# OSU-NLP-Group/saev

Hardware: AMD Instinct MI355X
Metric: activations/sec (train step), d_in=1024 x32 k=32 (higher is better)
Workload: dtype f32 (encoder: fp16 MFMA first pass with a rigorous error margin, survivors recomputed exactly in fp32; all else fp32)

## Files before the change

### include/saev_amd.h

```cpp
#ifndef SAEV_AMD_H
#define SAEV_AMD_H

#include <stdint.h>

#ifdef __cplusplus
extern "C" {
#endif

#define SAEV_AMD_ABI_VERSION 12

typedef enum {
    SAEV_OK = 0,
    SAEV_INVALID_ARG = -1,
    SAEV_HIP_ERROR = -2,
    SAEV_UNSUPPORTED = -3,
    SAEV_NOT_BOUND = -4,
    SAEV_RCCL_ERROR = -5,
    SAEV_STALE_PARAMS = -6,
    SAEV_ROW_OVERFLOW = -7
} saev_status;

typedef struct {
    int32_t d_model;
    int32_t d_sae;
// ... 44 lines not shown
typedef struct saev_ctx saev_ctx;

typedef struct {
    int32_t struct_size;
    int32_t dw_route;
    int32_t aux_small_max;
    int32_t fwd_route;
    int32_t csc_route;
    int32_t fin_route;
    int32_t prep_route;
    int32_t aux_dense_route;
    int32_t aux_small_route;
    int32_t group_route;
    int32_t aux_split_route;
    int32_t aux_wide_route;
} saev_debug_cfg;

int saev_abi_version(void);
const char* saev_last_error(const saev_ctx* ctx);

int saev_create(const saev_cfg* cfg, int device, saev_ctx** out);
int saev_create_ex(const saev_cfg* cfg, const saev_debug_cfg* dbg, int device, saev_ctx** out);
void saev_destroy(saev_ctx* ctx);

typedef struct {
    int32_t struct_size;
    int32_t row_cap;
    double batch_momentum;
    int32_t list_cap;
    int32_t reserved;
// ... 140 lines not shown
```

### saev_amd/_lib.py

```python

from __future__ import annotations

import ctypes as C
import os
import pathlib

_HERE = pathlib.Path(__file__).resolve().parent
LIB_PATH = pathlib.Path(os.environ.get("SAEV_AMD_LIB", _HERE / "libsaev_amd.so"))

ABI_VERSION = 12


class SaevCfg(C.Structure):
    _fields_ = [
        ("d_model", C.c_int32), ("d_sae", C.c_int32), ("top_k", C.c_int32), ("k_aux", C.c_int32),
        ("alpha", C.c_float), ("dead_threshold_tokens", C.c_int64),
        ("normalize_w_dec", C.c_int32), ("remove_parallel_grads", C.c_int32),
        ("max_batch", C.c_int32), ("encoder_mode", C.c_int32), ("aux_dead_cap", C.c_int32),
        ("shard_world", C.c_int32), ("bound_mode", C.c_int32), ("max_backward_rows", C.c_int32),
        ("activation", C.c_int32),
    ]


class SaevDebugCfg(C.Structure):

    _fields_ = [(n, C.c_int32) for n in ("struct_size", "dw_route", "aux_small_max", "fwd_route", "csc_route", "fin_route", "prep_route", "aux_dense_route",
                                         "aux_small_route", "group_route", "aux_split_route", "aux_wide_route")]


class SaevLayout(C.Structure):
    _fields_ = [(n, C.c_int64) for n in ("off_W_dec", "off_b_dec", "off_W_enc", "off_b_enc", "n_total", "chunk_a", "chunk_b")]


class SaevStepStats(C.Structure):
    _fields_ = [
        ("mse", C.c_float), ("aux", C.c_float), ("l0", C.c_float), ("l1", C.c_float),
        ("grad_norm", C.c_float), ("upper", C.c_float), ("n_dead", C.c_int32),
        ("n_overflow_rows", C.c_int32), ("cand_max", C.c_int32), ("dense_route", C.c_int32), ("sse", C.c_double), ("sum_sq", C.c_double),
    ]


class SaevMuonCfg(C.Structure):
# ... 148 lines not shown
```

### saev_amd/csrc/ctx.hip

```cpp
#include <hip/hip_runtime.h>

#include <algorithm>
#include <cmath>
#include <cstdio>
#include <cstdlib>
#include <cstring>
#include <dlfcn.h>
#include <mutex>
#include <string>
#include <vector>

#include "kernels.h"

namespace {
constexpr int AUX_KSPLIT_MAX = 16;
constexpr int CAND_CAP = 4096;
constexpr int CAND_STRIDE = CAND_CAP + 256;
constexpr int TIMING_RING = 512;
constexpr int DEAD_LAG = 4;
constexpr int DEAD_RING = 16;
enum { AUX_NONE = 0, AUX_SMALL_DEVICE = 1, AUX_SMALL_HOST = 2, AUX_DENSE = 3 };
}

struct saev_ctx {
// ... 42 lines not shown
    float* dval_pairs = nullptr;
    double *sumsq_partials = nullptr, *sumsq_total = nullptr;
    bool wenc_sq_valid = false;
    float2* row_proj = nullptr;
    float* enc_sq = nullptr;
    bool row_proj_valid = false, tail_proj_in_adam = false;
    bool wenc_t_pending = false;
    int64_t* toks = nullptr;
    int32_t *fired = nullptr, *dead = nullptr;
    int32_t* flags = nullptr;
    int32_t *chunk_starts = nullptr, *part_starts = nullptr, *work_latent = nullptr;
    float *dW_encT = nullptr, *partials = nullptr, *db_partials = nullptr;
    bool dws_ok = false;
    int dws_rows = 0;
    bool dws_pairs = false;
    float *gS = nullptr, *xS = nullptr, *dvp = nullptr;
    float* xS_ov = nullptr;
    float* xS_bwd = nullptr;
    float* dval_rows = nullptr;
    bool dval_fwd = false;
    float* wn2 = nullptr;
    float* sq_wave = nullptr;
    int sq_wave_n = 0;
    bool wn2_fresh = false;
    bool dval_pairs_ready = false;
    bool fused_forward = false;
    bool fwd_slices = false;
    bool fwd_step = false;
    float* rs_part = nullptr;
    float* xS_c = nullptr;
// ... 284 lines not shown
    A(dW_encT, S * D); A(partials, (size_t)c->max_part * 2 * D); A(db_partials, c->max_part); A(row_proj, S); A(enc_sq, S);
    {
        const bool rows_only = c->dbg.dw_route == 1;
        c->dws_ok = !rows_only && !btk && D % DWS_SLICE == 0 && (uint64_t)S * D * 4ull < (1ull << 32) && MBB < (1l << 24) &&
                    (uint64_t)MBB * K < (1ull << 31);
    }
    c->fwd_slices = !btk && c->cfg.encoder_mode == SAEV_ENCODER_F16R && c->dbg.fwd_route == 0 && D % RS_SLICE == 0 &&
                    (uint64_t)S * 128ull < (1ull << 32) - 256ull && fused_supported(c->cfg);
    if (c->fwd_slices) {
        A(rs_part, (size_t)(D / RS_SLICE) * MB * REFINE_CAP); A(surv_rng, MB * RS_MAX_RANGES);
        c->rs_lat_range = (int)std::max<long>(RS_LAT_RANGE, ((S + RS_MAX_RANGES - 1) / RS_MAX_RANGES + 255) / 256 * 256);
        c->rs_n_ranges = (int)((S + c->rs_lat_range - 1) / c->rs_lat_range);
    }
    if (c->fwd_slices && !c->dws_ok) A(xS, MBB * D);
    if (c->dws_ok) {
        A(gS, MBB * D); A(xS, MBB * D); A(dvp, (size_t)(D / DWS_SLICE) * MBB * K);
        if (c->dbg.dw_route != 2 && decode_forms_dval((int)D, (int)K)) A(dval_rows, MB * K);
        A(pv, MBB * K); A(pv2, MBB * K); A(plat, MBB * K); A(cut_lat, (MBB * K + DWS_RUN - 1) / DWS_RUN); A(cut_list, 4 * (1 + (MBB * K + DWS_RUN - 1) / DWS_RUN)); A(lat_unused, S);
        if (c->dval_rows != nullptr && c->dbg.fin_route == 0) { A(wn2, S); A(sq_wave, (size_t)2 * dw_slices_waves((int)D, (int)(MBB * K))); }
    }
    A(colsum_partials, ((MBB + 63) / 64) * D);
    A(sumsq_partials, 2 * 1024 + (S + 3) / 4 + 8 + transpose_blocks((int)S, (int)D)); A(sumsq_total, 1);
    if (c->cfg.encoder_mode != SAEV_ENCODER_F32 || KA > 0) {
        c->Dp = (int)((D + 31) / 32 * 32);
        c->S_pad = (int)((S + 255) / 256 * 256);
        c->MB_pad = (int)((MB + 255) / 256 * 256);
        A(zero_bias, std::max(S, D)); A(aux_scales, 16); A(aux_sync, absmax_parts_max((int)MB));
    }
    if (c->cfg.encoder_mode != SAEV_ENCODER_F32) {
        A(xs, (size_t)c->MB_pad * 2 * c->Dp);
// ... 509 lines not shown
                if (c->fwd_step) {
                    RefineSlicesArgs rs{};
                    rs.surv_idx = c->surv_idx; rs.surv_cnt = c->surv_cnt; rs.surv_val = c->surv_val; rs.surv_rng = c->surv_rng;
                    rs.xS = c->xS_c; rs.WeS = c->stream_ok ? c->WeS : c->dW_encT; rs.b_enc = sc.b_enc; rs.part = c->rs_part;
                    rs.n_rows = n; rs.S = c->cfg.d_sae; rs.D = c->cfg.d_model;
                    rs.lat_range = c->rs_lat_range; rs.n_ranges = c->rs_n_ranges;
                    rs.enable_flag = flag; rs.enable_when = when;
                    HIPCHK(c, launch_refine_slices(rs, s));
                    sc.sum_part = c->rs_part; sc.sum_bias = sc.b_enc; sc.sum_n = c->cfg.d_model / RS_SLICE; sc.sum_plane = (size_t)n * REFINE_CAP;
                } else {
                    HIPCHK(c, launch_refine_exact(sc, s));
                }
                sc.row_margin = nullptr; sc.tau_max = nullptr;
                sc.cand_cnt = c->surv_cnt; sc.cand_val = c->surv_val; sc.cand_idx = c->surv_idx; sc.cand_cap = REFINE_CAP; sc.cand_stride = REFINE_CAP;
            }
            HIPCHK(c, launch_select_cand(sc, s));
            return SAEV_OK;
        };
        const bool predict = c->cfg.bound_mode != 0 && ng == 32 && c->cfg.encoder_mode != SAEV_ENCODER_F32;
        int32_t *bad1 = c->flags + 9, *run2 = c->flags + 10, *gate = c->flags + 11;
        if (predict) {
            HIPCHK(c, launch_heur_gate(c->heur_state, pre_flag, gate, s));
            HIPCHK(c, launch_encoder_init(c->cand_cnt, n, c->gmax, 0, s, c->tau_max));
            timing_begin(c, s);
            int rc = run_encoder(c, x, n, EPI_TOPK, nullptr, gate, 0, s, true);
            if (rc != SAEV_OK) return rc;
            timing_end(c, s);
            HIPCHK(c, launch_overflow_check(c->cand_cnt, n, CAND_CAP, gate, bad1, c->flags + 2, c->flags + 3, s, need_dense,
                                            nullptr, c->heur_state + 3, nullptr, pre_flag));
            rc = select_stage(bad1, 0, bad1, c->tau_max);
            if (rc != SAEV_OK) return rc;
// ... 829 lines not shown
        w.part_dec = c->partials; w.part_enc = c->partials + 2 * runs_cap * D;
        w.cut_lat = c->cut_lat; w.cut_list = c->cut_list;
        w.lat_unused = (all_rows && c->fused_step) ? c->lat_unused : nullptr;
        c->unused_valid = w.lat_unused != nullptr;
        w.row_proj = a.row_proj; w.project = a.project; w.enc_sq = a.enc_sq;
        w.clear_bitmap = a.clear_bitmap; w.clear_words = a.clear_words;
        w.have_dval = c->dval_pairs_ready ? 1 : 0;
        c->sq_wave_n = 0;
        if (c->dval_pairs_ready && c->wn2_fresh && part == 0) {
            w.wn2 = c->wn2;
            if (c->fused_step && all_rows && c->sq_wave != nullptr && c->dbg.fin_route != 2) {
                c->sq_wave_n = dw_slices_waves(D, (int)((long)n * K));
                w.sq_wave_dec = c->sq_wave; w.sq_wave_enc = c->sq_wave + c->sq_wave_n;
            }
        }
        HIPCHK(c, launch_dw_slices(w, (int)((long)n * K), part, s));
    } else {
        c->unused_valid = false;
        HIPCHK(c, launch_dw_rows(a, max_work, s));
    }
    if (c->aux_route == AUX_DENSE)
        HIPCHK(c, launch_scatter_add_dead(c->dead_list, c->n_dead_host, D, c->dWd, c->dWe, c->dbe, c->grads + c->off_W_dec,
                                          c->dW_encT, c->grads + c->off_b_enc, lat_lo, lat_hi, s,
                                          c->aux_dev_count ? c->flags + 4 : nullptr, part, a.row_proj, a.W_dec, a.project, a.enc_sq,
                                          c->unused_valid ? c->lat_unused : nullptr, c->sq_wave_n > 0 ? c->starts : nullptr));
    else if (c->aux_route != AUX_NONE)
        HIPCHK(c, launch_scatter_add_dead(c->dead_list, c->aux_mfma ? c->aux_ndp : AUX_SMALL_MAX, D, c->dWd, c->dWe, c->dbe, c->grads + c->off_W_dec,
                                          c->dW_encT, c->grads + c->off_b_enc, lat_lo, lat_hi, s, c->flags + 4, part,
                                          a.row_proj, a.W_dec, a.project, a.enc_sq, c->unused_valid ? c->lat_unused : nullptr,
                                          c->sq_wave_n > 0 ? c->starts : nullptr));
    if (ov && c->aux_route != AUX_NONE && part != 2 && lat_lo == 0)
// ... 549 lines not shown
```

### saev_amd/csrc/kernels.h

```cpp
#pragma once
#include <hip/hip_runtime.h>
#include <stdint.h>

#include <string>

#include "../../include/saev_amd.h"

enum { EPI_DENSE = 0, EPI_TOPK = 1 };

struct EncodeArgs {
    const float* x;
    const float* W_enc;
    const float* b_enc;
    int n_rows, D, S;
    int s_splits;
    float* h_out;
    int ngroups;
    int32_t* gmax;
    int gmax_stride;
    int32_t* cand_cnt;
    float* cand_val;
    int32_t* cand_idx;
    int cand_cap;
    int cand_stride;
// ... 50 lines not shown
    size_t sum_plane;
};
hipError_t launch_refine_exact(const SelectCandArgs& a, hipStream_t stream);
constexpr int REFINE_CAP = 512;
constexpr int RS_SLICE = 32;
constexpr int RS_ROWS_MAX = 8;
constexpr int RS_LAT_RANGE = 32768;
constexpr int RS_MAX_RANGES = 8;
struct RefineSlicesArgs {
    const int32_t* surv_idx; const int32_t* surv_cnt; float* surv_val; const int32_t* surv_rng;
    const float* xS; const float* WeS; const float* b_enc; float* part;
    int n_rows, S, D, lat_range, n_ranges;
    const int32_t* enable_flag; int enable_when;
};
hipError_t launch_refine_slices(const RefineSlicesArgs& a, hipStream_t stream);
hipError_t launch_select_cand(const SelectCandArgs& a, hipStream_t stream);
hipError_t launch_init_i32(int32_t* p, int32_t v, int n, hipStream_t stream);
hipError_t launch_encoder_init(int32_t* cand_cnt, int n_rows, int32_t* gmax, int n_gmax, hipStream_t stream,
                               int32_t* tau_max = nullptr, const int32_t* enable_flag = nullptr, int enable_when = 0);
hipError_t launch_pre_encode(int32_t* cand_cnt, int n_rows, int32_t* gmax, int n_gmax, const float* xnorm, int D,
                             const float* wg_part, int n_part, const float* scales, int32_t* pre_flag, float* wmax_prev,
                             float* margin, int32_t* flags1, hipStream_t stream);
hipError_t launch_heur_gate(float* state, const int32_t* pre_flag, int32_t* gate, hipStream_t stream);
hipError_t launch_heur_update(float* state, const int32_t* bad, const float* cand_mean, int k, const int32_t* gate,
                              hipStream_t stream);
hipError_t launch_step_zero(saev_step_stats* stats, float* upper, int32_t* flag0, hipStream_t stream);
hipError_t launch_wnorm_max(const float* W_encT, int S, int D, float* wg_scratch, float* wmax, hipStream_t stream);
hipError_t launch_f16r_scales(const float* xmax_part, int n_part, const float* wmax, float* scales, hipStream_t stream);
hipError_t launch_pow2_scale(const float* absmax, float* pair, hipStream_t stream);
hipError_t launch_center_stats(const float* x, const float* mu, int n, int D, float* xnorm, float* wg_absmax,
                               hipStream_t stream, const float* xmax = nullptr);
// ... 129 lines not shown
    float* part_dec;
    float* part_enc;
    int32_t* cut_lat;
    int32_t* cut_list;
    float2* row_proj;
    int project;
    float* enc_sq;
    uint32_t* clear_bitmap;
    int clear_words;
    int32_t* lat_unused;
    int have_dval;
    const float* wn2;
    float* sq_wave_dec;
    float* sq_wave_enc;
};
hipError_t launch_dw_slices(const DwSlicesArgs& a, int max_pairs, int part, hipStream_t stream);
int dw_slices_waves(int D, int max_pairs);
hipError_t launch_slice_major_copy(const float* g, const float* x, int n, int D, float* gS, float* xS, hipStream_t stream);
hipError_t launch_transpose(const float* in, float* out, int S, int D, hipStream_t stream, double* sq_part = nullptr);
int transpose_blocks(int S, int D);

hipError_t launch_colsum(const float* m, int n_rows, int D, float* partials, float* out, int accumulate,
                         const int32_t* k_dev, hipStream_t stream, long row_stride = 0, float out_scale = 1.0f,
                         int col_mult = 0);
hipError_t launch_colsum_absmax(const float* m, int n_rows, int D, float* partials, float* out, float* wg_scratch,
                                float* absmax_out, hipStream_t stream, float out_scale = 1.0f,
                                saev_step_stats* zero_stats = nullptr, int32_t* zero_flag = nullptr);

hipError_t launch_normalize_rows(float* W, int S, int D, hipStream_t stream, float* wn2 = nullptr);
hipError_t launch_rpg(float* gW, const float* W, int S, int D, hipStream_t stream, double* sq_partials = nullptr,
                      int project = 1);
// ... 329 lines not shown
```

### saev_amd/csrc/select.hip

```cpp
#include "common.h"
#include "kernels.h"

namespace {

constexpr int SD_THREADS = 256;

__device__ __forceinline__ int block_excl_scan_256(int v, int* lds_wave_tot, int& total) {
    const int lane = threadIdx.x & 63, w = threadIdx.x >> 6;
    int incl = v;
#pragma unroll
    for (int o = 1; o < 64; o <<= 1) {
        int n = __shfl_up(incl, o, 64);
        if (lane >= o) incl += n;
    }
    if (lane == 63) lds_wave_tot[w] = incl;
    __syncthreads();
    int base = 0, tot = 0;
#pragma unroll
    for (int i = 0; i < 4; ++i) {
        const int t = lds_wave_tot[i];
        if (i < w) base += t;
        tot += t;
    }
    total = tot;
// ... 392 lines not shown
#pragma unroll
                for (int u = 0; u < 8; ++u) sv += v[u];
            }
            for (; c < a.sum_n; ++c) sv += a.sum_part[(size_t)c * a.sum_plane + o];
            lv[j] = sv + a.sum_bias[ci[j]];
        }
        __asm__ volatile("" ::: "memory");
        cv = lv;
    }
    if (n <= 64 && a.row_margin == nullptr) select_small_row(a, row, n, cv, ci);
    else if (n <= 512) select_cand_row<8>(a, row, n, s_idx, s_val, cv, ci);
    else if (n <= 1024) select_cand_row<16>(a, row, n, s_idx, s_val, cv, ci);
    else if (n <= 2048) select_cand_row<32>(a, row, n, s_idx, s_val, cv, ci);
    else if constexpr (BIG) select_cand_row<64>(a, row, n, s_idx, s_val, cv, ci);
    else select_cand_row_stream(a, row, n, s_idx, s_val, cv, ci);
}

__global__ void init_i32_kernel(int32_t* p, int32_t v, int n) {
    const int i = blockIdx.x * blockDim.x + threadIdx.x;
    if (i < n) p[i] = v;
}

__global__ void encoder_init_kernel(int32_t* cand_cnt, int n_rows, int32_t* gmax, int n_gmax, int32_t* tau_max,
                                    const int32_t* enable_flag, int enable_when) {
    if (enable_flag != nullptr && (*enable_flag != 0) != (enable_when != 0)) return;
    const int i = blockIdx.x * blockDim.x + threadIdx.x;
    if (i < n_rows) cand_cnt[i] = 0;
    if (i < n_gmax) gmax[i] = INT32_MIN;
    if (tau_max != nullptr && i < n_rows) tau_max[i] = INT32_MIN;
}
// ... 447 lines not shown
    } else {
        state[4] = 0.f;
        if (*cand_mean > 3.f * (float)k) z += 0.002f;
    }
    state[0] = fminf(fmaxf(z, 0.5f), 3.5f);
}

}

hipError_t launch_select_dense(const SelectDenseArgs& a, hipStream_t stream) {
    if (a.n_rows <= 0) return hipSuccess;
    hipLaunchKernelGGL(select_dense_kernel, dim3(a.n_rows), dim3(SD_THREADS), 0, stream, a);
    return hipGetLastError();
}

hipError_t launch_select_cand(const SelectCandArgs& a, hipStream_t stream) {
    if (a.n_rows <= 0) return hipSuccess;
    if (a.cand_cap > 4096 || (a.sum_part != nullptr && a.cand_cap > REFINE_CAP)) return hipErrorInvalidValue;
    if (a.k > 32) hipLaunchKernelGGL(select_cand_kernel<true>, dim3((a.n_rows + 3) / 4), dim3(256), 0, stream, a);
    else hipLaunchKernelGGL(select_cand_kernel<false>, dim3((a.n_rows + 3) / 4), dim3(256), 0, stream, a);
    return hipGetLastError();
}

hipError_t launch_init_i32(int32_t* p, int32_t v, int n, hipStream_t stream) {
    if (n <= 0) return hipSuccess;
    hipLaunchKernelGGL(init_i32_kernel, dim3((n + 255) / 256), dim3(256), 0, stream, p, v, n);
    return hipGetLastError();
}

hipError_t launch_encoder_init(int32_t* cand_cnt, int n_rows, int32_t* gmax, int n_gmax, hipStream_t stream, int32_t* tau_max,
                               const int32_t* enable_flag, int enable_when) {
    const int n = n_rows > n_gmax ? n_rows : n_gmax;
    if (n <= 0) return hipSuccess;
    hipLaunchKernelGGL(encoder_init_kernel, dim3((n + 255) / 256), dim3(256), 0, stream, cand_cnt, n_rows, gmax, n_gmax, tau_max,
// ... 97 lines not shown
```

### saev_amd/csrc/sparse.hip

```cpp
#include "common.h"
#include "kernels.h"

namespace {

template <int NV>
__device__ __forceinline__ void gather_rows_accum(f32x4 (&acc)[NV], const float* __restrict__ W, int D, int D4,
                                                  const int32_t* idx_row, const float* val_row, int k, int limit,
                                                  int lane) {
    for (int j0 = 0; j0 < k; j0 += 64) {
        const int cnt = min(64, k - j0);
        int32_t my_i = -1;
        float my_v = 0.f;
        if (lane < cnt) { my_i = idx_row[j0 + lane]; my_v = val_row[j0 + lane]; }
#pragma unroll 4
        for (int jj = 0; jj < cnt; ++jj) {
            const int32_t i = __shfl(my_i, jj, 64);
            const float v = __shfl(my_v, jj, 64);
            if (i < 0 || i >= limit) continue;
            const f32x4* wr = reinterpret_cast<const f32x4*>(W + (size_t)i * D);
#pragma unroll
            for (int n = 0; n < NV; ++n) {
                const int q = lane + 64 * n;
                if (q < D4) {
                    const f32x4 w = wr[q];
// ... 859 lines not shown
__global__ __launch_bounds__(256) void slice_major_copy_kernel(const float* __restrict__ g, const float* __restrict__ x, int n, int D,
                                                               float* __restrict__ gS, float* __restrict__ xS) {
    const int lane = threadIdx.x & 63;
    const int row = blockIdx.x * 4 + (threadIdx.x >> 6);
    if (row >= n) return;
    const f32x4* gr = reinterpret_cast<const f32x4*>(g + (size_t)row * D);
    const f32x4* xr = reinterpret_cast<const f32x4*>(x + (size_t)row * D);
    for (int q = lane; q < (D >> 2); q += 64) {
        const size_t o = ((size_t)(q >> 3) * n + row) * 8 + (q & 7);
        reinterpret_cast<f32x4*>(gS)[o] = gr[q];
        reinterpret_cast<f32x4*>(xS)[o] = xr[q];
    }
}

template <bool DEC, bool DVAL = true>
__global__ __launch_bounds__(256, (DEC && DVAL) ? 4 : 5) void dw_slices_kernel(DwSlicesArgs a, int wg_per_slice) {
    constexpr bool PASS_A = DEC && DVAL;
    constexpr int L = DWS_RUN;
    const int lane = threadIdx.x & 63, gi = lane >> 3, li = lane & 7;
    const int xcd = blockIdx.x & 7, q = blockIdx.x >> 3;
    const int slice = xcd + 8 * (q / wg_per_slice);
    const bool sq_on = (DEC ? a.sq_wave_dec : a.sq_wave_enc) != nullptr;
    auto sq_slot = [&]() -> float* {
        return (DEC ? a.sq_wave_dec : a.sq_wave_enc) + ((size_t)blockIdx.x * 4 + __builtin_amdgcn_readfirstlane((int)(threadIdx.x >> 6)));
    };
    if (slice * DWS_SLICE >= a.D) { if (sq_on && lane == 0) *sq_slot() = 0.f; return; }
    const int NP = a.starts[a.S];
    const int run0 = ((q % wg_per_slice) * 4 + (threadIdx.x >> 6)) * 8;
    if (run0 * L >= NP) { if (sq_on && lane == 0) *sq_slot() = 0.f; return; }
    const int run = run0 + gi;
    const int col = slice * DWS_SLICE + li * 4;
    const uint32_t colb = (uint32_t)col * 4u, rowb = (uint32_t)a.D * 4u, li16 = (uint32_t)li * 16u;
    auto bound = [&](int r) -> int {
        const long nb = (long)r * L;
        if (nb >= NP) return NP;
        const int lat = a.plat[nb];
        const int s = a.starts[lat];
        return (a.starts[lat + 1] - s < L) ? s : (int)nb;
    };
    const int p0 = bound(run), p1 = bound(run + 1);
    const bool live = p0 < p1;
    const int2* const pv = DEC ? a.pv : a.pv2;
    float* const out = DEC ? a.dW_dec : a.dW_encT;
    float* const part = DEC ? a.part_dec : a.part_enc;
    f32x4 acc = {0.f, 0.f, 0.f, 0.f};
    f32x4 w4 = {0.f, 0.f, 0.f, 0.f};
    float* const dvp = PASS_A ? a.dvp + (size_t)slice * a.pair_cap : nullptr;
    __shared__ float sh_sq[256];
    sh_sq[threadIdx.x] = 0.f;
    const int sel = (lane & 56) << 2;
    const __amdgpu_buffer_rsrc_t mres = __builtin_amdgcn_make_buffer_rsrc(
        const_cast<float*>(DEC ? a.gS : a.xS) + (size_t)slice * a.n_rows * DWS_SLICE * (DEC && a.P > 1 ? a.P : 1), 0,
        (uint32_t)a.n_rows * 128u * (uint32_t)(DEC && a.P > 1 ? a.P : 1), 0x00020000);
    const __amdgpu_buffer_rsrc_t wres = __builtin_amdgcn_make_buffer_rsrc(const_cast<float*>(a.W_dec), 0, (uint32_t)a.S * rowb, 0x00020000);

    auto load_info = [&](int t, int2& e, int& lat) {
        const int p = p0 + 8 * t + li;
        e = int2{0, 0};
        lat = 0;
        if (p < p1) {
            const i32x2 v = reinterpret_cast<const i32x2*>(pv)[p];
            e = int2{v[0], v[1]};
            lat = a.plat[p];
            if (p == p1 - 1) e.x |= DWS_END;
            if (p == p0) e.x &= ~DWS_FIRST;
        }
    };
    constexpr int PB = 4;
    auto issue = [&](const int2& e, int lat, int j0, int (&xj)[PB], int (&lj)[PB], f32x4 (&gt)[PB], f32x4 (&wt)[PB]) {
#pragma unroll
        for (int j = 0; j < PB; ++j) {
            xj[j] = __builtin_amdgcn_ds_bpermute(sel + 4 * (j0 + j), e.x);
            lj[j] = __builtin_amdgcn_ds_bpermute(sel + 4 * (j0 + j), lat);
            gt[j] = buf_load16(mres, ((uint32_t)xj[j] & ~127u) | li16);
            if (PASS_A && (xj[j] & DWS_FIRST)) wt[j] = buf_load16(wres, (uint32_t)lj[j] * rowb + colb);
        }
    };
    auto consume = [&](const int2& e, int j0, const int (&xc)[PB], const int (&lc)[PB], const f32x4 (&gc)[PB], const f32x4 (&wc)[PB],
                       const f32x4& wnext0, bool& head_open, float& dmine) {
        float vc[PB];
#pragma unroll
        for (int j = 0; j < PB; ++j) vc[j] = __int_as_float(__builtin_amdgcn_ds_bpermute(sel + 4 * (j0 + j), e.y));
#pragma unroll
        for (int j = 0; j < PB; ++j) {
            if (PASS_A) {
                float d = gc[j][0] * w4[0] + gc[j][1] * w4[1] + gc[j][2] * w4[2] + gc[j][3] * w4[3];
                d = group8_sum(d);
                dmine = li == j0 + j ? d : dmine;
            }
            acc += vc[j] * gc[j];
            if (xc[j] & (DWS_LAST | DWS_END)) {
                float* o;
                if (head_open) o = part + ((size_t)run * 2 + 0) * a.D + col;
                else if (!(xc[j] & DWS_LAST)) o = part + ((size_t)run * 2 + 1) * a.D + col;
                else {
                    o = out + (size_t)lc[j] * a.D + col;
                    if (sq_on)
                        sh_sq[threadIdx.x] += __builtin_fmaf(acc[3], acc[3], __builtin_fmaf(acc[2], acc[2], __builtin_fmaf(acc[1], acc[1], acc[0] * acc[0])));
                }
                *reinterpret_cast<f32x4*>(o) = acc;
                if (DEC && slice == 0 && li == 0 && (xc[j] & DWS_END)) {
                    const int cl = (!head_open && !(xc[j] & DWS_LAST)) ? lc[j] : -1;
                    a.cut_lat[run] = cl;
                    if (cl >= 0 && a.cut_list != nullptr)
                        reinterpret_cast<i32x4*>(a.cut_list)[1 + atomicAdd(&a.cut_list[0], 1)] = i32x4{run, cl, a.starts[cl], a.starts[cl + 1]};
                }
                head_open = false;
                acc = f32x4{0.f, 0.f, 0.f, 0.f};
                if (PASS_A) w4 = j + 1 < PB ? wc[j + 1 < PB ? j + 1 : 0] : wnext0;
            }
        }
    };
    int2 e_c, e_n;
    int lat_c, lat_n;
    int xa[PB], xb[PB], la[PB], lb[PB];
    f32x4 ga[PB], gb[PB], wa[PB], wb[PB];
    bool head_open = false;
    load_info(0, e_c, lat_c);
    if (live) {
        head_open = (pv[p0].x & DWS_FIRST) == 0;
        if (PASS_A) w4 = buf_load16(wres, (uint32_t)a.plat[p0] * rowb + colb);
    }
    issue(e_c, lat_c, 0, xa, la, ga, wa);
    load_info(1, e_n, lat_n);
#pragma unroll 1
    for (int t = 0; __any(p0 + 8 * t < p1); ++t) {
        float dmine = 0.f;
        issue(e_c, lat_c, PB, xb, lb, gb, wb);
        consume(e_c, 0, xa, la, ga, wa, wb[0], head_open, dmine);
        issue(e_n, lat_n, 0, xa, la, ga, wa);
        consume(e_c, PB, xb, lb, gb, wb, wa[0], head_open, dmine);
        if (PASS_A && p0 + 8 * t + li < p1) dvp[p0 + 8 * t + li] = dmine;
        e_c = e_n; lat_c = lat_n;
        load_info(t + 2, e_n, lat_n);
    }
    if (sq_on) {
        const float sq = wave_sum(sh_sq[threadIdx.x]);
        if (lane == 0) *sq_slot() = sq;
    }
}

__global__ __launch_bounds__(256) void dw_dval_sum_kernel(DwSlicesArgs a) {
    const int NP = a.starts[a.S];
    const int p = blockIdx.x * 256 + threadIdx.x;
    if (p >= NP) return;
    const int n_slices = a.D / DWS_SLICE;
    float s = 0.f;
    for (int c = 0; c < n_slices; ++c) s += a.dvp[(size_t)c * a.pair_cap + p];
    const int2 e = a.pv[p];
    const int b = a.P > 1 ? (e.x >> 7) % a.n_rows : (e.x >> 7);
    a.pv2[p] = int2{(b << 7) | (e.x & 127), __float_as_int(s)};
    if (a.clear_bitmap != nullptr) a.clear_bitmap[(size_t)a.plat[p] * a.clear_words + (b >> 5)] = 0u;
}
// ... 644 lines not shown
hipError_t launch_dw_rows(const DwRowsArgs& a, int max_work, hipStream_t stream) {
    return dispatch_nv(a.D, [&](auto nv) {
        hipLaunchKernelGGL(dw_rows_kernel<decltype(nv)::value>, dim3((max_work + 3) / 4), dim3(256), 0, stream, a);
        hipLaunchKernelGGL(dw_combine_kernel<decltype(nv)::value>, dim3((a.lat_hi - a.lat_lo + 3) / 4, 2), dim3(256), 0, stream, a);
    });
}
hipError_t launch_slice_major_copy(const float* g, const float* x, int n, int D, float* gS, float* xS, hipStream_t stream) {
    if (n <= 0) return hipSuccess;
    hipLaunchKernelGGL(slice_major_copy_kernel, dim3((n + 3) / 4), dim3(256), 0, stream, g, x, n, D, gS, xS);
    return hipGetLastError();
}
int dw_slices_waves(int D, int max_pairs) {
    const int n_runs = (max_pairs + DWS_RUN - 1) / DWS_RUN;
    return ((D / DWS_SLICE + 7) / 8) * 8 * ((n_runs + 31) / 32) * 4;
}
hipError_t launch_dw_slices(const DwSlicesArgs& a_in, int max_pairs, int part, hipStream_t stream) {
    DwSlicesArgs a = a_in;
    if (a.D % DWS_SLICE != 0 || max_pairs <= 0) return hipErrorInvalidValue;
    const int n_runs = (max_pairs + DWS_RUN - 1) / DWS_RUN;
    const int wg_per_slice = (n_runs + 31) / 32;
    const int grid = ((a.D / DWS_SLICE + 7) / 8) * 8 * wg_per_slice;
    const bool light = part == 0 && a.have_dval && a.wn2 != nullptr;
    if (!light) { a.sq_wave_dec = nullptr; a.sq_wave_enc = nullptr; }
    if (part != 2 && a.have_dval) {
        hipLaunchKernelGGL((dw_slices_kernel<true, false>), dim3(grid), dim3(256), 0, stream, a, wg_per_slice);
        if (a.clear_bitmap != nullptr && !light) hipLaunchKernelGGL(dw_clear_bitmap_kernel, dim3((max_pairs + 255) / 256), dim3(256), 0, stream, a);
    } else if (part != 2) {
        hipLaunchKernelGGL(dw_slices_kernel<true>, dim3(grid), dim3(256), 0, stream, a, wg_per_slice);
        hipLaunchKernelGGL(dw_dval_sum_kernel, dim3((max_pairs + 255) / 256), dim3(256), 0, stream, a);
    }
    if (part != 1) hipLaunchKernelGGL(dw_slices_kernel<false>, dim3(grid), dim3(256), 0, stream, a, wg_per_slice);
    const int kinds = part == 0 ? 2 : 1, kind0 = part == 2 ? 1 : 0;
    if (light) {
        const int n_cut = a.cut_list != nullptr ? std::min(2 * (n_runs - 1), 8192) : 0;
        if (a.cut_list == nullptr && n_runs > 1) return hipErrorInvalidValue;
        return dispatch_nv(a.D, [&](auto nv) {
            hipLaunchKernelGGL(dw_finalize_light_kernel<decltype(nv)::value>, dim3(n_cut + (a.S + 31) / 32), dim3(256), 0, stream, a, n_cut);
        });
    }
    return dispatch_nv(a.D, [&](auto nv) {
        if (n_runs > 1) hipLaunchKernelGGL(dw_finalize_cut_kernel<decltype(nv)::value>, dim3(n_runs - 1, kinds), dim3(256), 0, stream, a, kind0);
        hipLaunchKernelGGL(dw_finalize_kernel<decltype(nv)::value>, dim3((a.S + 3) / 4, kinds), dim3(256), 0, stream, a, kind0);
    });
}
hipError_t launch_transpose(const float* in, float* out, int S, int D, hipStream_t stream, double* sq_part) {
    hipLaunchKernelGGL(transpose_kernel, dim3((S + 63) / 64, (D + 63) / 64), dim3(256), 0, stream, in, out, S, D, sq_part);
// ... 26 lines not shown
```

### saev_amd/engine.py

```python

from __future__ import annotations

import ctypes as C
import dataclasses
import math
import os

import torch

from . import _lib


DEFAULT_ENCODER = "f16r"


@dataclasses.dataclass(frozen=True)
class EngineConfig:
    d_model: int
    d_sae: int
    top_k: int = 32
    k_aux: int = 512
    alpha: float = 1.0 / 32.0
    dead_threshold_tokens: int = 10_000_000
    normalize_w_dec: bool = True
# ... 3 lines not shown
    shard_world: int = 1
    max_backward_rows: int = 0
    bounds: str = dataclasses.field(default_factory=lambda: os.environ.get("SAEV_AMD_BOUNDS", "guaranteed"))
    encoder: str = dataclasses.field(default_factory=lambda: os.environ.get("SAEV_AMD_ENCODER", DEFAULT_ENCODER))
    dw_route: str = dataclasses.field(default_factory=lambda: os.environ.get("SAEV_AMD_DW", "slices"))
    fwd_route: str = dataclasses.field(default_factory=lambda: os.environ.get("SAEV_AMD_FWD", "default"))
    aux_small_max: int = dataclasses.field(default_factory=lambda: int(os.environ.get("SAEV_AMD_AUX_SMALL_MAX", "0")))
    csc_route: int = dataclasses.field(default_factory=lambda: int(os.environ.get("SAEV_AMD_CSC", "0")))
    fin_route: int = dataclasses.field(default_factory=lambda: int(os.environ.get("SAEV_AMD_FIN", "0")))
    prep_route: int = dataclasses.field(default_factory=lambda: int(os.environ.get("SAEV_AMD_PREP", "0")))
    aux_dense_route: int = dataclasses.field(default_factory=lambda: int(os.environ.get("SAEV_AMD_AUX_DENSE", "0")))
    aux_small_route: int = dataclasses.field(default_factory=lambda: int(os.environ.get("SAEV_AMD_AUX_SMALL", "0")))
    group_route: int = dataclasses.field(default_factory=lambda: int(os.environ.get("SAEV_AMD_GROUP", "0")))
    aux_split_route: int = dataclasses.field(default_factory=lambda: int(os.environ.get("SAEV_AMD_AUX_SPLIT", "0")))
    aux_wide_route: int = dataclasses.field(default_factory=lambda: int(os.environ.get("SAEV_AMD_AUX_WIDE", "0")))
    activation: str = "topk"
    row_cap: int = 0
    batch_momentum: float = 0.1
    select_list_cap: int = 0


@dataclasses.dataclass(frozen=True)
class MuonConfig:

    weight_decay: float = 0.1
    momentum: float = 0.95
    nesterov: bool = True
    ns_coefficients: tuple[float, float, float] = (3.4445, -4.7750, 2.0315)
    eps: float = 1e-07
    ns_steps: int = 5
# ... 295 lines not shown
    def _create_ctx(self) -> None:
        cfg, S, D = self.cfg, self.cfg.d_sae, self.cfg.d_model
        ccfg = _lib.SaevCfg(
            d_model=D, d_sae=S, top_k=cfg.top_k, k_aux=cfg.k_aux, alpha=cfg.alpha,
            dead_threshold_tokens=cfg.dead_threshold_tokens,
            normalize_w_dec=int(cfg.normalize_w_dec), remove_parallel_grads=int(cfg.remove_parallel_grads),
            max_batch=cfg.max_batch, encoder_mode={"f32": 0, "f16x3": 1, "bf16": 2, "f16r": 3}[cfg.encoder],
            aux_dead_cap=cfg.aux_dead_cap, shard_world=cfg.shard_world,
            bound_mode={"guaranteed": 0, "predicted": 1}[cfg.bounds], max_backward_rows=cfg.max_backward_rows,
            activation={"topk": _lib.ACT_TOPK, "relu": _lib.ACT_RELU, "batch_topk": _lib.ACT_BATCHTOPK}[cfg.activation],
        )
        dbg = _lib.SaevDebugCfg(
            struct_size=C.sizeof(_lib.SaevDebugCfg), dw_route={"slices": 0, "rows": 1, "slices_a": 2}[cfg.dw_route],
            aux_small_max=cfg.aux_small_max, fwd_route={"default": 0, "rows": 1}[cfg.fwd_route],
            csc_route=cfg.csc_route, fin_route=cfg.fin_route, prep_route=cfg.prep_route, aux_dense_route=cfg.aux_dense_route, aux_small_route=cfg.aux_small_route,
            group_route=cfg.group_route, aux_split_route=cfg.aux_split_route, aux_wide_route=cfg.aux_wide_route)
        ctx = C.c_void_p()
        if cfg.activation == "batch_topk":
            bt = _lib.SaevBatchTopKCfg(struct_size=C.sizeof(_lib.SaevBatchTopKCfg), row_cap=cfg.row_cap, batch_momentum=cfg.batch_momentum,
                                       list_cap=cfg.select_list_cap)
            rc = self.lib.saev_create_batch_topk(C.byref(ccfg), C.byref(dbg), C.byref(bt), self.device.index, C.byref(ctx))
        else:
            rc = self.lib.saev_create_ex(C.byref(ccfg), C.byref(dbg), self.device.index, C.byref(ctx))
        if rc != 0:
            raise _lib.SaevError(f"saev_create failed with status {rc} for {cfg}")
        self.ctx = ctx
        self._chk(self.lib.saev_bind(ctx, _ptr(self.params), _ptr(self.grads), _ptr(self.adam_m), _ptr(self.adam_v)), "saev_bind")
        self._chk(self.lib.saev_bind_tracker(ctx, _ptr(self.toks_since_active), _ptr(self.fired)), "saev_bind_tracker")
        self._chk(self.lib.saev_bind_sumsq(ctx, _ptr(self.sumsq)), "saev_bind_sumsq")
        if self._w_enc_t is not None:
            self._chk(self.lib.saev_bind_w_enc_t(ctx, _ptr(self._w_enc_t)), "saev_bind_w_enc_t")
# ... 490 lines not shown
```

Before: 6.301 million.

## Make dW slice kernels persistent with prefetched work items; add lean final select kernel

The dW slice kernels now launch only as many workgroups as can be resident, sized by an occupancy query at context creation, and loop over work items. Each wave prefetches the next item's run boundaries and pair info in stages interleaved with the current item's accumulation loop. This hides the latency of the dependent boundary lookups and cuts launch-tail waste. Separately, candidate selection gets a lean kernel that sums partial planes into shared memory without the margin or overflow handling. Both are default-on behind a new walk_route debug switch, and the debug struct gains a field without an ABI version bump.

```diff
diff --git a/include/saev_amd.h b/include/saev_amd.h
--- a/include/saev_amd.h
+++ b/include/saev_amd.h
@@ -82,6 +82,7 @@
     int32_t group_route;
     int32_t aux_split_route;
     int32_t aux_wide_route;
+    int32_t walk_route;
 } saev_debug_cfg;
 
 int saev_abi_version(void);
diff --git a/saev_amd/_lib.py b/saev_amd/_lib.py
--- a/saev_amd/_lib.py
+++ b/saev_amd/_lib.py
@@ -25,7 +25,7 @@
 class SaevDebugCfg(C.Structure):
 
     _fields_ = [(n, C.c_int32) for n in ("struct_size", "dw_route", "aux_small_max", "fwd_route", "csc_route", "fin_route", "prep_route", "aux_dense_route",
-                                         "aux_small_route", "group_route", "aux_split_route", "aux_wide_route")]
+                                         "aux_small_route", "group_route", "aux_split_route", "aux_wide_route", "walk_route")]
 
 
 class SaevLayout(C.Structure):
diff --git a/saev_amd/csrc/ctx.hip b/saev_amd/csrc/ctx.hip
--- a/saev_amd/csrc/ctx.hip
+++ b/saev_amd/csrc/ctx.hip
@@ -80,6 +80,7 @@
     bool dws_ok = false;
     int dws_rows = 0;
     bool dws_pairs = false;
+    int dws_resident[3] = {0, 0, 0};
     float *gS = nullptr, *xS = nullptr, *dvp = nullptr;
     float* xS_ov = nullptr;
     float* xS_bwd = nullptr;
@@ -394,6 +395,7 @@
     }
     if (c->fwd_slices && !c->dws_ok) A(xS, MBB * D);
     if (c->dws_ok) {
+        for (int w = 0; w < 3; ++w) c->dws_resident[w] = dw_slices_resident(w);
         A(gS, MBB * D); A(xS, MBB * D); A(dvp, (size_t)(D / DWS_SLICE) * MBB * K);
         if (c->dbg.dw_route != 2 && decode_forms_dval((int)D, (int)K)) A(dval_rows, MB * K);
         A(pv, MBB * K); A(pv2, MBB * K); A(plat, MBB * K); A(cut_lat, (MBB * K + DWS_RUN - 1) / DWS_RUN); A(cut_list, 4 * (1 + (MBB * K + DWS_RUN - 1) / DWS_RUN)); A(lat_unused, S);
@@ -933,7 +935,7 @@
                 sc.row_margin = nullptr; sc.tau_max = nullptr;
                 sc.cand_cnt = c->surv_cnt; sc.cand_val = c->surv_val; sc.cand_idx = c->surv_idx; sc.cand_cap = REFINE_CAP; sc.cand_stride = REFINE_CAP;
             }
-            HIPCHK(c, launch_select_cand(sc, s));
+            HIPCHK(c, launch_select_cand(sc, s, c->dbg.walk_route == 0));
             return SAEV_OK;
         };
         const bool predict = c->cfg.bound_mode != 0 && ng == 32 && c->cfg.encoder_mode != SAEV_ENCODER_F32;
@@ -1793,7 +1795,7 @@
                 w.sq_wave_dec = c->sq_wave; w.sq_wave_enc = c->sq_wave + c->sq_wave_n;
             }
         }
-        HIPCHK(c, launch_dw_slices(w, (int)((long)n * K), part, s));
+        HIPCHK(c, launch_dw_slices(w, (int)((long)n * K), part, s, c->dbg.walk_route == 0 ? c->dws_resident : nullptr));
     } else {
         c->unused_valid = false;
         HIPCHK(c, launch_dw_rows(a, max_work, s));
diff --git a/saev_amd/csrc/kernels.h b/saev_amd/csrc/kernels.h
--- a/saev_amd/csrc/kernels.h
+++ b/saev_amd/csrc/kernels.h
@@ -88,7 +88,7 @@
     const int32_t* enable_flag; int enable_when;
 };
 hipError_t launch_refine_slices(const RefineSlicesArgs& a, hipStream_t stream);
-hipError_t launch_select_cand(const SelectCandArgs& a, hipStream_t stream);
+hipError_t launch_select_cand(const SelectCandArgs& a, hipStream_t stream, bool lean_final = false);
 hipError_t launch_init_i32(int32_t* p, int32_t v, int n, hipStream_t stream);
 hipError_t launch_encoder_init(int32_t* cand_cnt, int n_rows, int32_t* gmax, int n_gmax, hipStream_t stream,
                                int32_t* tau_max = nullptr, const int32_t* enable_flag = nullptr, int enable_when = 0);
@@ -248,7 +248,8 @@
     float* sq_wave_dec;
     float* sq_wave_enc;
 };
-hipError_t launch_dw_slices(const DwSlicesArgs& a, int max_pairs, int part, hipStream_t stream);
+hipError_t launch_dw_slices(const DwSlicesArgs& a, int max_pairs, int part, hipStream_t stream, const int* resident = nullptr);
+int dw_slices_resident(int which);
 int dw_slices_waves(int D, int max_pairs);
 hipError_t launch_slice_major_copy(const float* g, const float* x, int n, int D, float* gS, float* xS, hipStream_t stream);
 hipError_t launch_transpose(const float* in, float* out, int S, int D, hipStream_t stream, double* sq_part = nullptr);
diff --git a/saev_amd/csrc/select.hip b/saev_amd/csrc/select.hip
--- a/saev_amd/csrc/select.hip
+++ b/saev_amd/csrc/select.hip
@@ -430,6 +430,43 @@
     else if (n <= 2048) select_cand_row<32>(a, row, n, s_idx, s_val, cv, ci);
     else if constexpr (BIG) select_cand_row<64>(a, row, n, s_idx, s_val, cv, ci);
     else select_cand_row_stream(a, row, n, s_idx, s_val, cv, ci);
+}
+
+__global__ __launch_bounds__(256) void select_final_kernel(SelectCandArgs a) {
+    if (a.enable_flag != nullptr && (*a.enable_flag != 0) != (a.enable_when != 0)) return;
+    __shared__ int32_t s_idx[4][64];
+    __shared__ float s_val[4][64];
+    __shared__ float l_sum[4][REFINE_CAP];
+    const int row = blockIdx.x * 4 + (threadIdx.x >> 6);
+    if (row >= a.n_rows) return;
+    const int n = min(a.cand_cnt[row], a.cand_cap);
+    const int32_t* ci = a.cand_idx + (size_t)row * a.cand_stride;
+    float* const lv = l_sum[threadIdx.x >> 6];
+    for (int j = threadIdx.x & 63; j < n; j += 64) {
+        const float* sp = a.sum_part + (size_t)row * a.cand_stride + j;
+        const float bias = a.sum_bias[ci[j]];
+        float sv = 0.f;
+        int c = 0;
+        for (; c + 32 <= a.sum_n; c += 32) {
+            float v[32];
+#pragma unroll
+            for (int u = 0; u < 32; ++u) v[u] = sp[(size_t)(c + u) * a.sum_plane];
+#pragma unroll
+            for (int u = 0; u < 32; ++u) sv += v[u];
+        }
+        for (; c + 8 <= a.sum_n; c += 8) {
+            float v[8];
+#pragma unroll
+            for (int u = 0; u < 8; ++u) v[u] = sp[(size_t)(c + u) * a.sum_plane];
+#pragma unroll
+            for (int u = 0; u < 8; ++u) sv += v[u];
+        }
+        for (; c < a.sum_n; ++c) sv += sp[(size_t)c * a.sum_plane];
+        lv[j] = sv + bias;
+    }
+    __asm__ volatile("" ::: "memory");
+    if (n <= 64) select_small_row(a, row, n, lv, ci);
+    else select_cand_row<8>(a, row, n, s_idx, s_val, lv, ci);
 }
 
 __global__ void init_i32_kernel(int32_t* p, int32_t v, int n) {
@@ -907,10 +944,12 @@
     return hipGetLastError();
 }
 
-hipError_t launch_select_cand(const SelectCandArgs& a, hipStream_t stream) {
+hipError_t launch_select_cand(const SelectCandArgs& a, hipStream_t stream, bool lean_final) {
     if (a.n_rows <= 0) return hipSuccess;
     if (a.cand_cap > 4096 || (a.sum_part != nullptr && a.cand_cap > REFINE_CAP)) return hipErrorInvalidValue;
-    if (a.k > 32) hipLaunchKernelGGL(select_cand_kernel<true>, dim3((a.n_rows + 3) / 4), dim3(256), 0, stream, a);
+    if (lean_final && a.sum_part != nullptr && a.row_margin == nullptr && a.ovf == nullptr && a.k <= 32)
+        hipLaunchKernelGGL(select_final_kernel, dim3((a.n_rows + 3) / 4), dim3(256), 0, stream, a);
+    else if (a.k > 32) hipLaunchKernelGGL(select_cand_kernel<true>, dim3((a.n_rows + 3) / 4), dim3(256), 0, stream, a);
     else hipLaunchKernelGGL(select_cand_kernel<false>, dim3((a.n_rows + 3) / 4), dim3(256), 0, stream, a);
     return hipGetLastError();
 }
diff --git a/saev_amd/csrc/sparse.hip b/saev_amd/csrc/sparse.hip
--- a/saev_amd/csrc/sparse.hip
+++ b/saev_amd/csrc/sparse.hip
@@ -897,129 +897,174 @@
 }
 
 template <bool DEC, bool DVAL = true>
-__global__ __launch_bounds__(256, (DEC && DVAL) ? 4 : 5) void dw_slices_kernel(DwSlicesArgs a, int wg_per_slice) {
+__global__ __launch_bounds__(256, (DEC && DVAL) ? 4 : 5) void dw_slices_kernel(DwSlicesArgs a, int wg_per_slice, int items) {
     constexpr bool PASS_A = DEC && DVAL;
+    constexpr bool WALK = !PASS_A;
     constexpr int L = DWS_RUN;
     const int lane = threadIdx.x & 63, gi = lane >> 3, li = lane & 7;
-    const int xcd = blockIdx.x & 7, q = blockIdx.x >> 3;
-    const int slice = xcd + 8 * (q / wg_per_slice);
+    const int xcd = blockIdx.x & 7, walk = gridDim.x >> 3;
+    const int wave = __builtin_amdgcn_readfirstlane((int)(threadIdx.x >> 6));
     const bool sq_on = (DEC ? a.sq_wave_dec : a.sq_wave_enc) != nullptr;
-    auto sq_slot = [&]() -> float* {
-        return (DEC ? a.sq_wave_dec : a.sq_wave_enc) + ((size_t)blockIdx.x * 4 + __builtin_amdgcn_readfirstlane((int)(threadIdx.x >> 6)));
-    };
-    if (slice * DWS_SLICE >= a.D) { if (sq_on && lane == 0) *sq_slot() = 0.f; return; }
+    auto sq_slot = [&](int q) -> float* { return (DEC ? a.sq_wave_dec : a.sq_wave_enc) + (((size_t)q * 8 + xcd) * 4 + wave); };
     const int NP = a.starts[a.S];
-    const int run0 = ((q % wg_per_slice) * 4 + (threadIdx.x >> 6)) * 8;
-    if (run0 * L >= NP) { if (sq_on && lane == 0) *sq_slot() = 0.f; return; }
-    const int run = run0 + gi;
-    const int col = slice * DWS_SLICE + li * 4;
-    const uint32_t colb = (uint32_t)col * 4u, rowb = (uint32_t)a.D * 4u, li16 = (uint32_t)li * 16u;
-    auto bound = [&](int r) -> int {
-        const long nb = (long)r * L;
-        if (nb >= NP) return NP;
-        const int lat = a.plat[nb];
-        const int s = a.starts[lat];
-        return (a.starts[lat + 1] - s < L) ? s : (int)nb;
-    };
-    const int p0 = bound(run), p1 = bound(run + 1);
-    const bool live = p0 < p1;
+    const uint32_t rowb = (uint32_t)a.D * 4u, li16 = (uint32_t)li * 16u;
     const int2* const pv = DEC ? a.pv : a.pv2;
     float* const out = DEC ? a.dW_dec : a.dW_encT;
     float* const part = DEC ? a.part_dec : a.part_enc;
-    f32x4 acc = {0.f, 0.f, 0.f, 0.f};
-    f32x4 w4 = {0.f, 0.f, 0.f, 0.f};
-    float* const dvp = PASS_A ? a.dvp + (size_t)slice * a.pair_cap : nullptr;
     __shared__ float sh_sq[256];
-    sh_sq[threadIdx.x] = 0.f;
     const int sel = (lane & 56) << 2;
-    const __amdgpu_buffer_rsrc_t mres = __builtin_amdgcn_make_buffer_rsrc(
-        const_cast<float*>(DEC ? a.gS : a.xS) + (size_t)slice * a.n_rows * DWS_SLICE * (DEC && a.P > 1 ? a.P : 1), 0,
-        (uint32_t)a.n_rows * 128u * (uint32_t)(DEC && a.P > 1 ? a.P : 1), 0x00020000);
     const __amdgpu_buffer_rsrc_t wres = __builtin_amdgcn_make_buffer_rsrc(const_cast<float*>(a.W_dec), 0, (uint32_t)a.S * rowb, 0x00020000);
 
-    auto load_info = [&](int t, int2& e, int& lat) {
-        const int p = p0 + 8 * t + li;
-        e = int2{0, 0};
-        lat = 0;
-        if (p < p1) {
-            const i32x2 v = reinterpret_cast<const i32x2*>(pv)[p];
-            e = int2{v[0], v[1]};
-            lat = a.plat[p];
+    int q_n = 0, slice_n = 0, run0_n = 0, stage = 3;
+    bool valid_n = false;
+    int pf[4] = {0, 0, 0, 0};
+    auto pf_start = [&](int q) {
+        q_n = q; stage = 3; valid_n = false;
+        if (q < items) {
+            slice_n = xcd + 8 * (q / wg_per_slice);
+            run0_n = ((q % wg_per_slice) * 4 + wave) * 8;
+            valid_n = slice_n * DWS_SLICE < a.D && (long)run0_n * L < NP;
+            if (valid_n) stage = 0;
+        }
+    };
+    auto pf_step = [&]() {
+        if (stage == 0) {
+            const long nb = (long)(run0_n + gi + (li == 7 ? 1 : 0)) * L;
+            pf[0] = nb < NP ? a.plat[nb] : 0;
+            stage = 1;
+        } else if (stage == 1) {
+            pf[1] = a.starts[pf[0]];
+            pf[2] = a.starts[pf[0] + 1];
+            stage = 2;
+        } else if (stage == 2) {
+            const long nb = (long)(run0_n + gi + (li == 7 ? 1 : 0)) * L;
+            const int bnd = nb >= NP ? NP : ((pf[2] - pf[1] < L) ? pf[1] : (int)nb);
+            const int p = __builtin_amdgcn_ds_bpermute(sel, bnd) + li, p1 = __builtin_amdgcn_ds_bpermute(sel + 28, bnd);
+            pf[0] = bnd; pf[1] = 0; pf[2] = 0; pf[3] = 0;
+            if (p < p1) {
+                const i32x2 v = reinterpret_cast<const i32x2*>(pv)[p];
+                pf[1] = v[0]; pf[2] = v[1];
+                pf[3] = a.plat[p];
+            }
+            stage = 3;
+        }
+    };
+    auto pf_finish = [&]() { while (stage < 3) pf_step(); };
+    pf_start(blockIdx.x >> 3);
+    pf_finish();
+#pragma unroll 1
+    while (q_n < items) {
+        const int q = q_n, slice = slice_n, run = run0_n + gi;
+        const bool valid = valid_n;
+        const int p0 = __builtin_amdgcn_ds_bpermute(sel, pf[0]), p1 = __builtin_amdgcn_ds_bpermute(sel + 28, pf[0]);
+        int2 e_c = int2{pf[1], pf[2]}, e_n;
+        int lat_c = pf[3], lat_n;
+        if constexpr (WALK) pf_start(q + walk);
+        else { q_n = items; stage = 3; valid_n = false; }
+        if (!valid) {
+            if (sq_on && lane == 0) *sq_slot(q) = 0.f;
+            pf_finish();
+            continue;
+        }
+        const bool live = p0 < p1;
+        const int col = slice * DWS_SLICE + li * 4;
+        const uint32_t colb = (uint32_t)col * 4u;
+        f32x4 acc = {0.f, 0.f, 0.f, 0.f};
+        f32x4 w4 = {0.f, 0.f, 0.f, 0.f};
+        float* const dvp = PASS_A ? a.dvp + (size_t)slice * a.pair_cap : nullptr;
+        sh_sq[threadIdx.x] = 0.f;
+        const __amdgpu_buffer_rsrc_t mres = __builtin_amdgcn_make_buffer_rsrc(
+            const_cast<float*>(DEC ? a.gS : a.xS) + (size_t)slice * a.n_rows * DWS_SLICE * (DEC && a.P > 1 ? a.P : 1), 0,
+            (uint32_t)a.n_rows * 128u * (uint32_t)(DEC && a.P > 1 ? a.P : 1), 0x00020000);
+
+        auto mark = [&](int p, int2& e) {
             if (p == p1 - 1) e.x |= DWS_END;
             if (p == p0) e.x &= ~DWS_FIRST;
-        }
-    };
-    constexpr int PB = 4;
-    auto issue = [&](const int2& e, int lat, int j0, int (&xj)[PB], int (&lj)[PB], f32x4 (&gt)[PB], f32x4 (&wt)[PB]) {
-#pragma unroll
-        for (int j = 0; j < PB; ++j) {
-            xj[j] = __builtin_amdgcn_ds_bpermute(sel + 4 * (j0 + j), e.x);
-            lj[j] = __builtin_amdgcn_ds_bpermute(sel + 4 * (j0 + j), lat);
-            gt[j] = buf_load16(mres, ((uint32_t)xj[j] & ~127u) | li16);
-            if (PASS_A && (xj[j] & DWS_FIRST)) wt[j] = buf_load16(wres, (uint32_t)lj[j] * rowb + colb);
-        }
-    };
-    auto consume = [&](const int2& e, int j0, const int (&xc)[PB], const int (&lc)[PB], const f32x4 (&gc)[PB], const f32x4 (&wc)[PB],
-                       const f32x4& wnext0, bool& head_open, float& dmine) {
-        float vc[PB];
-#pragma unroll
-        for (int j = 0; j < PB; ++j) vc[j] = __int_as_float(__builtin_amdgcn_ds_bpermute(sel + 4 * (j0 + j), e.y));
-#pragma unroll
-        for (int j = 0; j < PB; ++j) {
-            if (PASS_A) {
-                float d = gc[j][0] * w4[0] + gc[j][1] * w4[1] + gc[j][2] * w4[2] + gc[j][3] * w4[3];
-                d = group8_sum(d);
-                dmine = li == j0 + j ? d : dmine;
-            }
-            acc += vc[j] * gc[j];
-            if (xc[j] & (DWS_LAST | DWS_END)) {
-                float* o;
-                if (head_open) o = part + ((size_t)run * 2 + 0) * a.D + col;
-                else if (!(xc[j] & DWS_LAST)) o = part + ((size_t)run * 2 + 1) * a.D + col;
-                else {
-                    o = out + (size_t)lc[j] * a.D + col;
-                    if (sq_on)
-                        sh_sq[threadIdx.x] += __builtin_fmaf(acc[3], acc[3], __builtin_fmaf(acc[2], acc[2], __builtin_fmaf(acc[1], acc[1], acc[0] * acc[0])));
+        };
+        auto load_info = [&](int t, int2& e, int& lat) {
+            const int p = p0 + 8 * t + li;
+            e = int2{0, 0};
+            lat = 0;
+            if (p < p1) {
+                const i32x2 v = reinterpret_cast<const i32x2*>(pv)[p];
+                e = int2{v[0], v[1]};
+                lat = a.plat[p];
+                mark(p, e);
+            }
+        };
+        constexpr int PB = 4;
+        auto issue = [&](const int2& e, int lat, int j0, int (&xj)[PB], f32x4 (&gt)[PB], f32x4 (&wt)[PB]) {
+#pragma unroll
+            for (int j = 0; j < PB; ++j) {
+                xj[j] = __builtin_amdgcn_ds_bpermute(sel + 4 * (j0 + j), e.x);
+                gt[j] = buf_load16(mres, ((uint32_t)xj[j] & ~127u) | li16);
+                if (PASS_A && (xj[j] & DWS_FIRST))
+                    wt[j] = buf_load16(wres, (uint32_t)__builtin_amdgcn_ds_bpermute(sel + 4 * (j0 + j), lat) * rowb + colb);
+            }
+        };
+        auto consume = [&](const int2& e, int lat, int j0, const int (&xc)[PB], const f32x4 (&gc)[PB], const f32x4 (&wc)[PB],
+                           const f32x4& wnext0, bool& head_open, float& dmine) {
+            float vc[PB];
+#pragma unroll
+            for (int j = 0; j < PB; ++j) vc[j] = __int_as_float(__builtin_amdgcn_ds_bpermute(sel + 4 * (j0 + j), e.y));
+#pragma unroll
+            for (int j = 0; j < PB; ++j) {
+                if (PASS_A) {
+                    float d = gc[j][0] * w4[0] + gc[j][1] * w4[1] + gc[j][2] * w4[2] + gc[j][3] * w4[3];
+                    d = group8_sum(d);
+                    dmine = li == j0 + j ? d : dmine;
                 }
-                *reinterpret_cast<f32x4*>(o) = acc;
-                if (DEC && slice == 0 && li == 0 && (xc[j] & DWS_END)) {
-                    const int cl = (!head_open && !(xc[j] & DWS_LAST)) ? lc[j] : -1;
-                    a.cut_lat[run] = cl;
-                    if (cl >= 0 && a.cut_list != nullptr)
-                        reinterpret_cast<i32x4*>(a.cut_list)[1 + atomicAdd(&a.cut_list[0], 1)] = i32x4{run, cl, a.starts[cl], a.starts[cl + 1]};
+                acc += vc[j] * gc[j];
+                if (xc[j] & (DWS_LAST | DWS_END)) {
+                    const int lcj = __builtin_amdgcn_ds_bpermute(sel + 4 * (j0 + j), lat);
+                    float* o;
+                    if (head_open) o = part + ((size_t)run * 2 + 0) * a.D + col;
+                    else if (!(xc[j] & DWS_LAST)) o = part + ((size_t)run * 2 + 1) * a.D + col;
+                    else {
+                        o = out + (size_t)lcj * a.D + col;
+                        if (sq_on)
+                            sh_sq[threadIdx.x] += __builtin_fmaf(acc[3], acc[3], __builtin_fmaf(acc[2], acc[2], __builtin_fmaf(acc[1], acc[1], acc[0] * acc[0])));
+                    }
+                    *reinterpret_cast<f32x4*>(o) = acc;
+                    if (DEC && slice == 0 && li == 0 && (xc[j] & DWS_END)) {
+                        const int cl = (!head_open && !(xc[j] & DWS_LAST)) ? lcj : -1;
+                        a.cut_lat[run] = cl;
+                        if (cl >= 0 && a.cut_list != nullptr)
+                            reinterpret_cast<i32x4*>(a.cut_list)[1 + atomicAdd(&a.cut_list[0], 1)] = i32x4{run, cl, a.starts[cl], a.starts[cl + 1]};
+                    }
+                    head_open = false;
+                    acc = f32x4{0.f, 0.f, 0.f, 0.f};
+                    if (PASS_A) w4 = j + 1 < PB ? wc[j + 1 < PB ? j + 1 : 0] : wnext0;
                 }
-                head_open = false;
-                acc = f32x4{0.f, 0.f, 0.f, 0.f};
-                if (PASS_A) w4 = j + 1 < PB ? wc[j + 1 < PB ? j + 1 : 0] : wnext0;
-            }
-        }
-    };
-    int2 e_c, e_n;
-    int lat_c, lat_n;
-    int xa[PB], xb[PB], la[PB], lb[PB];
-    f32x4 ga[PB], gb[PB], wa[PB], wb[PB];
-    bool head_open = false;
-    load_info(0, e_c, lat_c);
-    if (live) {
-        head_open = (pv[p0].x & DWS_FIRST) == 0;
-        if (PASS_A) w4 = buf_load16(wres, (uint32_t)a.plat[p0] * rowb + colb);
-    }
-    issue(e_c, lat_c, 0, xa, la, ga, wa);
-    load_info(1, e_n, lat_n);
+            }
+        };
+        int xa[PB], xb[PB];
+        f32x4 ga[PB], gb[PB], wa[PB], wb[PB];
+        bool head_open = false;
+        if (live) {
+            head_open = (__builtin_amdgcn_ds_bpermute(sel, e_c.x) & DWS_FIRST) == 0;
+            if (PASS_A) w4 = buf_load16(wres, (uint32_t)__builtin_amdgcn_ds_bpermute(sel, lat_c) * rowb + colb);
+        }
+        if (p0 + li < p1) mark(p0 + li, e_c);
+        issue(e_c, lat_c, 0, xa, ga, wa);
+        load_info(1, e_n, lat_n);
 #pragma unroll 1
-    for (int t = 0; __any(p0 + 8 * t < p1); ++t) {
-        float dmine = 0.f;
-        issue(e_c, lat_c, PB, xb, lb, gb, wb);
-        consume(e_c, 0, xa, la, ga, wa, wb[0], head_open, dmine);
-        issue(e_n, lat_n, 0, xa, la, ga, wa);
-        consume(e_c, PB, xb, lb, gb, wb, wa[0], head_open, dmine);
-        if (PASS_A && p0 + 8 * t + li < p1) dvp[p0 + 8 * t + li] = dmine;
-        e_c = e_n; lat_c = lat_n;
-        load_info(t + 2, e_n, lat_n);
-    }
-    if (sq_on) {
-        const float sq = wave_sum(sh_sq[threadIdx.x]);
-        if (lane == 0) *sq_slot() = sq;
+        for (int t = 0; __any(p0 + 8 * t < p1); ++t) {
+            float dmine = 0.f;
+            issue(e_c, lat_c, PB, xb, gb, wb);
+            consume(e_c, lat_c, 0, xa, ga, wa, wb[0], head_open, dmine);
+            pf_step();
+            issue(e_n, lat_n, 0, xa, ga, wa);
+            consume(e_c, lat_c, PB, xb, gb, wb, wa[0], head_open, dmine);
+            if (PASS_A && p0 + 8 * t + li < p1) dvp[p0 + 8 * t + li] = dmine;
+            e_c = e_n; lat_c = lat_n;
+            load_info(t + 2, e_n, lat_n);
+        }
+        pf_finish();
+        if (sq_on) {
+            const float sq = wave_sum(sh_sq[threadIdx.x]);
+            if (lane == 0) *sq_slot(q) = sq;
+        }
     }
 }
 
@@ -1694,22 +1739,34 @@
     const int n_runs = (max_pairs + DWS_RUN - 1) / DWS_RUN;
     return ((D / DWS_SLICE + 7) / 8) * 8 * ((n_runs + 31) / 32) * 4;
 }
-hipError_t launch_dw_slices(const DwSlicesArgs& a_in, int max_pairs, int part, hipStream_t stream) {
+int dw_slices_resident(int which) {
+    int dev = 0, cus = 0, per_cu = 0;
+    if (hipGetDevice(&dev) != hipSuccess || hipDeviceGetAttribute(&cus, hipDeviceAttributeMultiprocessorCount, dev) != hipSuccess) return 0;
+    const hipError_t e = which == 0 ? hipOccupancyMaxActiveBlocksPerMultiprocessor(&per_cu, dw_slices_kernel<true, false>, 256, 0)
+                       : which == 1 ? hipOccupancyMaxActiveBlocksPerMultiprocessor(&per_cu, dw_slices_kernel<true, true>, 256, 0)
+                                    : hipOccupancyMaxActiveBlocksPerMultiprocessor(&per_cu, dw_slices_kernel<false, true>, 256, 0);
+    return e == hipSuccess ? per_cu * cus : 0;
+}
+hipError_t launch_dw_slices(const DwSlicesArgs& a_in, int max_pairs, int part, hipStream_t stream, const int* resident) {
     DwSlicesArgs a = a_in;
     if (a.D % DWS_SLICE != 0 || max_pairs <= 0) return hipErrorInvalidValue;
     const int n_runs = (max_pairs + DWS_RUN - 1) / DWS_RUN;
     const int wg_per_slice = (n_runs + 31) / 32;
-    const int grid = ((a.D / DWS_SLICE + 7) / 8) * 8 * wg_per_slice;
+    const int items = ((a.D / DWS_SLICE + 7) / 8) * wg_per_slice;
+    auto grid_of = [&](int which) {
+        const int r = resident != nullptr && which != 1 ? resident[which] / 8 : 0;
+        return 8 * (r > 0 ? std::min(r, items) : items);
+    };
     const bool light = part == 0 && a.have_dval && a.wn2 != nullptr;
     if (!light) { a.sq_wave_dec = nullptr; a.sq_wave_enc = nullptr; }
     if (part != 2 && a.have_dval) {
-        hipLaunchKernelGGL((dw_slices_kernel<true, false>), dim3(grid), dim3(256), 0, stream, a, wg_per_slice);
+        hipLaunchKernelGGL((dw_slices_kernel<true, false>), dim3(grid_of(0)), dim3(256), 0, stream, a, wg_per_slice, items);
         if (a.clear_bitmap != nullptr && !light) hipLaunchKernelGGL(dw_clear_bitmap_kernel, dim3((max_pairs + 255) / 256), dim3(256), 0, stream, a);
     } else if (part != 2) {
-        hipLaunchKernelGGL(dw_slices_kernel<true>, dim3(grid), dim3(256), 0, stream, a, wg_per_slice);
+        hipLaunchKernelGGL(dw_slices_kernel<true>, dim3(grid_of(1)), dim3(256), 0, stream, a, wg_per_slice, items);
         hipLaunchKernelGGL(dw_dval_sum_kernel, dim3((max_pairs + 255) / 256), dim3(256), 0, stream, a);
     }
-    if (part != 1) hipLaunchKernelGGL(dw_slices_kernel<false>, dim3(grid), dim3(256), 0, stream, a, wg_per_slice);
+    if (part != 1) hipLaunchKernelGGL(dw_slices_kernel<false>, dim3(grid_of(2)), dim3(256), 0, stream, a, wg_per_slice, items);
     const int kinds = part == 0 ? 2 : 1, kind0 = part == 2 ? 1 : 0;
     if (light) {
         const int n_cut = a.cut_list != nullptr ? std::min(2 * (n_runs - 1), 8192) : 0;
diff --git a/saev_amd/engine.py b/saev_amd/engine.py
--- a/saev_amd/engine.py
+++ b/saev_amd/engine.py
@@ -41,6 +41,7 @@
     group_route: int = dataclasses.field(default_factory=lambda: int(os.environ.get("SAEV_AMD_GROUP", "0")))
     aux_split_route: int = dataclasses.field(default_factory=lambda: int(os.environ.get("SAEV_AMD_AUX_SPLIT", "0")))
     aux_wide_route: int = dataclasses.field(default_factory=lambda: int(os.environ.get("SAEV_AMD_AUX_WIDE", "0")))
+    walk_route: int = dataclasses.field(default_factory=lambda: int(os.environ.get("SAEV_AMD_WALK", "0")))
     activation: str = "topk"
     row_cap: int = 0
     batch_momentum: float = 0.1
@@ -366,7 +367,7 @@
             struct_size=C.sizeof(_lib.SaevDebugCfg), dw_route={"slices": 0, "rows": 1, "slices_a": 2}[cfg.dw_route],
             aux_small_max=cfg.aux_small_max, fwd_route={"default": 0, "rows": 1}[cfg.fwd_route],
             csc_route=cfg.csc_route, fin_route=cfg.fin_route, prep_route=cfg.prep_route, aux_dense_route=cfg.aux_dense_route, aux_small_route=cfg.aux_small_route,
-            group_route=cfg.group_route, aux_split_route=cfg.aux_split_route, aux_wide_route=cfg.aux_wide_route)
+            group_route=cfg.group_route, aux_split_route=cfg.aux_split_route, aux_wide_route=cfg.aux_wide_route, walk_route=cfg.walk_route)
         ctx = C.c_void_p()
         if cfg.activation == "batch_topk":
             bt = _lib.SaevBatchTopKCfg(struct_size=C.sizeof(_lib.SaevBatchTopKCfg), row_cap=cfg.row_cap, batch_momentum=cfg.batch_momentum,
```

Measured after the change: 6.209 million. -1.5%, worse.
